# javahedi/SpinDynamics.jl

Hardware: AMD Instinct MI355X
Metric: H|psi> matvecs/s, XXZ L=32 Sz=0 (higher is better)
Workload: dtype c128

## Files before the change

profiles/l2_model.py:

```python
#!/usr/bin/env python3
import os
import sys
from collections import OrderedDict
from math import comb

import numpy as np

L = int(sys.argv[1]) if len(sys.argv) > 1 else 28
orders = sys.argv[2:] or ["lex", "chunk", "orbit"]
LS, nup = int(os.environ.get("LS", "12")), L // 2
p = L - LS
CAP = int(float(os.environ.get("CAP_MIB", "4")) * (1 << 20))
W = int(os.environ.get("W", "160"))
LO, HI = int(os.environ.get("LO", "513")), int(os.environ.get("HI", "1024"))


def tile_len(P):
    return comb(LS, nup - bin(P).count("1")) if 0 <= nup - bin(P).count("1") <= LS else 0


def n_up_first(P):
    t = nup - bin(P).count("1")
    return comb(LS - 1, t - 1) if t >= 1 else 0


all_tiles = [P for P in range(1 << p) if LO <= tile_len(P) <= HI]


def canon(P, FO, greedy):
    C0, member, ng, b = P, 0, 0, 1
    while b + 1 <= p and ng < FO:
        if ((P >> (b - 1)) ^ (P >> b)) & 1:
            if not (P >> (b - 1)) & 1:
                C0 ^= 3 << (b - 1)
                member |= 1 << ng
            ng += 1
            b += 2
        else:
            b += 1 if greedy else 2
    return C0, member


def order_orbit(tiles, FO=6, greedy=False, OC=1, gray=False):
    first, keys = {}, []
    for P in tiles:
        C0, mem = canon(P, FO, greedy)
        if C0 not in first:
            first[C0] = len(first)
        if gray:
            mem = mem ^ (mem >> 1)
        keys.append((first[C0], mem))
    idx = sorted(range(len(tiles)), key=lambda k: keys[k])
    q = [[] for _ in range(8)]
    o, k = 0, 0
    while k < len(idx):
        e = k
        while e < len(idx) and keys[idx[e]][0] == keys[idx[k]][0]:
            e += 1
        q[(o // OC) % 8].extend(tiles[i] for i in idx[k:e])
        o += 1
        k = e
    return q


def order_chunk(tiles, CH=32):
    q = [[] for _ in range(8)]
    for c in range(0, len(tiles), CH):
        q[(c // CH) % 8].extend(tiles[c:c + CH])
    return q


def order_lex(tiles):
    return [tiles[x::8] for x in range(8)]


def events(queue):
    ev = []
    life = 1.0
    for j, P in enumerate(queue):
        t0 = j * life / W
        reads = [((P, 0), n_up_first(P) * 16), ((P, 1), (tile_len(P) - n_up_first(P)) * 16)]
        for b in range(1, p):
            if ((P >> (b - 1)) ^ (P >> b)) & 1:
                Q = P ^ (3 << (b - 1))
                reads.append(((Q, 0), n_up_first(Q) * 16))
                reads.append(((Q, 1), (tile_len(Q) - n_up_first(Q)) * 16))
        Q = P ^ (1 << (p - 1))
        if tile_len(Q) > 0:
            half = 0 if (P >> (p - 1)) & 1 else 1
            sz = n_up_first(Q) * 16 if half == 0 else (tile_len(Q) - n_up_first(Q)) * 16
            if sz > 0:
                reads.append(((Q, half), sz))
        n = len(reads)
        for k, (obj, sz) in enumerate(reads):
            ev.append((t0 + life * (k // 2) / (n // 2 + 1), obj, sz))
    return ev


class LRU:
    def __init__(self, cap):
        self.cap, self.used, self.d = cap, 0, OrderedDict()

    def access(self, obj, sz):
        if obj in self.d:
            self.d.move_to_end(obj)
            return True
        self.d[obj] = sz
        self.used += sz
        while self.used > self.cap:
            _, s2 = self.d.popitem(last=False)
            self.used -= s2
        return False


def simulate(queue):
    ev = events(queue)
    ev.sort(key=lambda e: e[0])
    l2, req, miss = LRU(CAP), 0, 0
    for _, obj, sz in ev:
        req += sz
        if not l2.access(obj, sz):
            miss += sz
    return req, miss


def simulate_all(queues, mall_bytes):
    ev = []
    for x, q in enumerate(queues):
        ev.extend((t, x, obj, sz) for (t, obj, sz) in events(q))
    ev.sort(key=lambda e: e[0])
    l2 = [LRU(CAP) for _ in queues]
    mall = LRU(mall_bytes)
    req = m2 = m3 = 0
    for _, x, obj, sz in ev:
        req += sz
        if l2[x].access(obj, sz):
            continue
        m2 += sz
        if not mall.access(obj, sz):
            m3 += sz
    return req, m2, m3


def parse(name):
    if name == "lex":
        return order_lex(all_tiles)
    if name.startswith("chunk"):
        return order_chunk(all_tiles, int(name[5:] or 32))
    if name.startswith("orbit") or name.startswith("greedy") or name.startswith("gray"):
        kind = "greedy" if name.startswith("greedy") else ("gray" if name.startswith("gray") else "orbit")
        rest = name[len(kind):]
        FO, OC = 6, 1
        if rest:
            parts = rest.split("x")
            FO = int(parts[0])
            if len(parts) > 1:
                OC = int(parts[1])
        return order_orbit(all_tiles, FO, kind == "greedy", OC, kind == "gray")
    raise SystemExit("unknown order " + name)


print(f"L={L} p={p} tiles in class: {len(all_tiles)}  rows: {sum(tile_len(P) for P in all_tiles)}")
MALL = float(os.environ.get("MALL_MIB", "0"))
for name in orders:
    q = parse(name)
    if MALL > 0:
        r, m2, m3 = simulate_all(q, int(MALL * (1 << 20)))
        rows = sum(tile_len(P) for x in q for P in x)
        print(f"{name:12s} read requests {r / rows:6.1f} B/row   L2 misses {m2 / rows:6.1f} B/row   memory-side misses {m3 / rows:6.1f} B/row", flush=True)
        continue
    tot_req = tot_miss = 0
    for x in (0, 3):
        r, m_ = simulate(q[x])
        tot_req += r
        tot_miss += m_
    rows = sum(tile_len(P) for P in q[0]) + sum(tile_len(P) for P in q[3])
    print(f"{name:12s} read requests {tot_req / rows:6.1f} B/row   L2 misses {tot_miss / rows:6.1f} B/row   hit {1 - tot_miss / tot_req:.3f}", flush=True)
```

spindynamics.jl_amd/csrc/basis.cpp:

```cpp
#include <algorithm>
#include <cmath>
#include <cstdlib>
#include <cstring>

#include "sd_internal.hpp"

int64_t sd_binom(int n, int k) {
  if (k < 0 || k > n || n < 0) return 0;
  if (k > n - k) k = n - k;
  __int128 r = 1;
  for (int i = 1; i <= k; ++i) r = r * (n - k + i) / i;
  return (int64_t)r;
}

void sd_fill_binom(std::vector<int64_t> &tab) {
  const int W = SD_MAX_L + 1;
  tab.assign((size_t)W * W, 0);
  for (int n = 0; n < W; ++n)
    for (int k = 0; k <= n; ++k) tab[(size_t)n * W + k] = sd_binom(n, k);
}

static inline int64_t B(const sd_model *m, int n, int k) {
  if (k < 0 || n < 0 || k > n) return 0;
  return m->binom[(size_t)n * (SD_MAX_L + 1) + k];
}

uint64_t sd_unrank_host(const sd_model *m, int64_t idx0) {
  if (m->nup < 0) return (uint64_t)idx0;
  uint64_t s = 0;
  int r = m->nup;
  for (int k = 1; k <= m->L && r > 0; ++k) {
    int64_t c = B(m, m->L - k, r - 1);
    if (idx0 < c) { s |= (uint64_t)1 << (k - 1); --r; }
    else idx0 -= c;
  }
  return s;
}

int64_t sd_rank_host(const sd_model *m, uint64_t s) {
  if (m->L < 64 && (s >> m->L) != 0) return -1;
  if (m->nup < 0) return (int64_t)s;
  if (__builtin_popcountll(s) != m->nup) return -1;
  int64_t idx = 0;
  int r = m->nup;
  for (int k = 1; k <= m->L && r > 0; ++k) {
    if ((s >> (k - 1)) & 1) --r;
    else idx += B(m, m->L - k, r - 1);
  }
  return idx;
}

static void enum_sector(int n, int t, std::vector<uint16_t> &out) {
  if (t < 0 || t > n) return;
  std::vector<int> c(t);
  for (int k = 0; k < t; ++k) c[k] = k + 1;
  for (;;) {
    uint32_t s = 0;
    for (int k = 0; k < t; ++k) s |= 1u << (c[k] - 1);
    out.push_back((uint16_t)s);
    int k = t - 1;
    while (k >= 0 && c[k] == n - t + k + 1) --k;
    if (k < 0) break;
    ++c[k];
    for (int q = k + 1; q < t; ++q) c[q] = c[q - 1] + 1;
  }
}

static int suffix_bits_from_env() {
  int ls = 12;
  if (const char *e = getenv("SD_SUFFIX_BITS")) ls = atoi(e);
  if (ls < 2) ls = 2;
  if (ls > 15) ls = 15;
  return ls;
}

static int64_t tile_base_global(const sd_model *m, uint32_t P) {
  int64_t idx = 0;
  int r = m->nup;
  for (int k = 1; k <= m->p && r > 0; ++k) {
    if ((P >> (k - 1)) & 1) --r;
    else idx += B(m, m->L - k, r - 1);
  }
  return idx;
}

struct TileRef { int64_t base; uint32_t P; };

static void collect_needs(const sd_model *m, const std::vector<TileRef> &tiles, const std::vector<int> &owner, int q,
                          int nn_hops, std::vector<uint8_t> &need) {
  const int p = m->p;
  for (size_t k = 0; k < tiles.size(); ++k) {
    if (owner[k] != q) continue;
    uint32_t P = tiles[k].P;
    if (nn_hops > 0) {
      for (int b = 1; b <= p - 1; ++b)
        if (((P >> (b - 1)) & 1) != ((P >> b) & 1)) need[P ^ (3u << (b - 1))] = 1;
      if (p >= 1) {
        uint32_t Q = P ^ (1u << (p - 1));
        int t2 = m->nup - __builtin_popcount(Q);
        if (t2 >= 0 && t2 <= m->LS) need[Q] = 1;
      }
    }
    for (size_t h = (size_t)nn_hops; h < m->hop_i.size(); ++h) {
      int i = m->hop_i[h], j = m->hop_j[h];
      bool ip = i <= p, jp = j <= p;
      uint32_t Q = P;
      if (ip && jp) {
        if (((P >> (i - 1)) & 1) == ((P >> (j - 1)) & 1)) continue;
        Q = P ^ (1u << (i - 1)) ^ (1u << (j - 1));
      } else if (ip) Q = P ^ (1u << (i - 1));
      else if (jp) Q = P ^ (1u << (j - 1));
      else continue;
      int t2 = m->nup - __builtin_popcount(Q);
      if (t2 >= 0 && t2 <= m->LS) need[Q] = 1;
    }
  }
}

static int count_nn_hops(const sd_model *m) {
  int L = m->L;
  if (L < 2 || (int)m->hop_i.size() < L - 1) return 0;
  for (int k = 0; k < L - 1; ++k)
    if (m->hop_i[k] != k + 1 || m->hop_j[k] != k + 2) return 0;
  return L - 1;
}

static const int XCD_FO_CLASSES = 5, XCD_FO_PACKED = 6;
static std::vector<std::vector<size_t>> xcd_queues(const sd_model *m, int p, const std::vector<uint32_t> &tp_io,
                                                   std::vector<int64_t> &first_seen, const int FO) {
  std::vector<std::vector<size_t>> q(8);
  {
    const int CH = 32;
    const size_t nt = tp_io.size();
    auto canon = [&](uint32_t P, int *member_out) {
      uint32_t C0 = P; int member = 0, ng = 0;
      for (int b = 1; b + 1 <= p && ng < FO; b += 2)
        if (((P >> (b - 1)) ^ (P >> b)) & 1u) {
          if (!((P >> (b - 1)) & 1u)) { C0 ^= 3u << (b - 1); member |= 1 << ng; }
          ++ng;
        }
      if (member_out) *member_out = member;
      return C0;
    };
    auto first_seen_reset = [&](uint32_t P) { first_seen[canon(P, nullptr)] = -1; };
    if (nt >= 64 && p >= 3 && count_nn_hops(m) > 0) {
      std::vector<uint64_t> key(nt);
      int64_t n_orb = 0;
      for (size_t k = 0; k < nt; ++k) {
        int member = 0;
        const uint32_t C0 = canon(tp_io[k], &member);
        if (first_seen[C0] < 0) first_seen[C0] = n_orb++;
        key[k] = ((uint64_t)first_seen[C0] << 8) | (uint64_t)member;
      }
      std::vector<size_t> idx(nt);
      for (size_t k = 0; k < nt; ++k) idx[k] = k;
      std::stable_sort(idx.begin(), idx.end(), [&](size_t a, size_t b) { return key[a] < key[b]; });
      size_t o = 0;
      for (size_t k = 0; k < nt;) {
        size_t e = k;
        while (e < nt && (key[idx[e]] >> 8) == (key[idx[k]] >> 8)) ++e;
        for (size_t t = k; t < e; ++t) q[o % 8].push_back(idx[t]);
        ++o; k = e;
      }
      for (size_t k = 0; k < nt; ++k) first_seen_reset(tp_io[k]);
    } else {
      const size_t group = (size_t)8 * CH, full = nt >= (size_t)16 * CH ? nt / group * group : 0;
      for (size_t b = 0; b < nt; ++b) {
        size_t t = b;
        if (b < full) {
          const size_t x = b % 8, sl = b / 8, g = sl / CH, i = sl % CH;
          t = g * group + x * CH + i;
        }
        q[b % 8].push_back(t);
      }
    }
  }
  return q;
}

static void xcd_order(const sd_model *m, int p, std::vector<uint32_t> &tp_io, std::vector<int64_t> &tb_io,
                      std::vector<int64_t> &first_seen) {
  const std::vector<std::vector<size_t>> q = xcd_queues(m, p, tp_io, first_seen, XCD_FO_CLASSES);
  const size_t nt = tp_io.size();
  std::vector<uint32_t> tp; std::vector<int64_t> tb;
  tp.reserve(nt); tb.reserve(nt);
  size_t longest = 0;
  for (auto &v : q) longest = std::max(longest, v.size());
  for (size_t j = 0; j < longest; ++j)
    for (int x = 0; x < 8; ++x)
      if (j < q[x].size()) { tp.push_back(tp_io[q[x][j]]); tb.push_back(tb_io[q[x][j]]); }
  tp_io.swap(tp); tb_io.swap(tb);
}

struct BisectPlan {
  int d = 0;
  int s[4] = {0, 0, 0, 0};
  int thr[3][4] = {{0}};
  double score = 1e300;
  double busiest = 0;
};

static int bisect_owner(const BisectPlan &bp, const int *k) {
  int cum[4] = {0, 0, 0, 0};
  for (int i = 0; i < bp.d; ++i) cum[i + 1] = cum[i] + k[i];
  int r = 0;
  for (int lev = 0; lev < bp.d; ++lev) r = 2 * r + (cum[bp.d - lev] > bp.thr[lev][r] ? 1 : 0);
  return r;
}

static bool eval_bisect(const sd_model *m, BisectPlan &bp) {
  const int d = bp.d, L = m->L, nup = m->nup, P = 1 << d;
  int len[3] = {0, 0, 0};
  for (int i = 0; i < d; ++i) len[i] = bp.s[i + 1] - bp.s[i];
  const int rest = L - bp.s[d];
  auto weight = [&](const int *k) {
    int sum = 0; double w = 1;
    for (int i = 0; i < d; ++i) { w *= (double)B(m, len[i], k[i]); sum += k[i]; }
    return w * (double)B(m, rest, nup - sum);
  };
  auto for_cells = [&](auto &&fn) {
    int k[3] = {0, 0, 0};
    for (k[0] = 0; k[0] <= len[0]; ++k[0])
      for (k[1] = 0; k[1] <= (d > 1 ? len[1] : 0); ++k[1])
        for (k[2] = 0; k[2] <= (d > 2 ? len[2] : 0); ++k[2]) fn(k);
  };
  for (int lev = 0; lev < d; ++lev)
    for (int pre = 0; pre < (1 << lev); ++pre) {
      const int blk = d - lev;
      std::vector<double> hist(bp.s[blk] + 1, 0.0);
      double tot = 0;
      for_cells([&](const int *k) {
        int cum[4] = {0, 0, 0, 0};
        for (int i = 0; i < d; ++i) cum[i + 1] = cum[i] + k[i];
        int r = 0;
        for (int q = 0; q < lev; ++q) r = 2 * r + (cum[d - q] > bp.thr[q][r] ? 1 : 0);
        if (r != pre) return;
        const double w = weight(k);
        hist[cum[blk]] += w; tot += w;
      });
      if (tot <= 0) return false;
      double acc = 0, bestd = 1e300; int t = 0;
      for (int v = 0; v < bp.s[blk]; ++v) {
        acc += hist[v];
        const double dd = std::fabs(acc - tot / 2);
        if (dd < bestd) { bestd = dd; t = v; }
      }
      bp.thr[lev][pre] = t;
    }
  std::vector<double> size(P, 0.0), vol(P, 0.0), pair((size_t)P * P, 0.0);
  for_cells([&](const int *k) {
    int sum = 0;
    for (int i = 0; i < d; ++i) sum += k[i];
    const int kr = nup - sum;
    if (kr < 0 || kr > rest) return;
    const int me = bisect_owner(bp, k);
    size[me] += weight(k);
    for (int i = 0; i < d; ++i) {
      const bool last = i == d - 1;
      const int lr = last ? rest : len[i + 1], kright = last ? kr : k[i + 1];
      double others = 1;
      for (int q = 0; q < d; ++q) if (q != i && (last || q != i + 1)) others *= (double)B(m, len[q], k[q]);
      if (!last) others *= (double)B(m, rest, kr);
      for (int dir = 0; dir < 2; ++dir) {
        const double n = dir == 0 ? (double)B(m, len[i] - 1, k[i] - 1) * (double)B(m, lr - 1, kright) * others
                                  : (double)B(m, len[i] - 1, k[i]) * (double)B(m, lr - 1, kright - 1) * others;
        if (n <= 0) continue;
        int k2[3] = {k[0], k[1], k[2]};
        k2[i] += dir == 0 ? -1 : 1;
        if (!last) k2[i + 1] += dir == 0 ? 1 : -1;
        const int o = bisect_owner(bp, k2);
        if (o != me) { vol[me] += n; pair[(size_t)me * P + o] += n; }
      }
    }
  });
  double tot = 0;
  for (int r = 0; r < P; ++r) tot += size[r];
  bp.score = 0; bp.busiest = 0;
  for (int r = 0; r < P; ++r) {
    if (size[r] <= 0 || size[r] > 1.15 * tot / P) return false;
    bp.score = std::max(bp.score, vol[r] / size[r]);
  }
  for (double v : pair) bp.busiest = std::max(bp.busiest, v);
  return true;
}

static bool best_bisect_plan(const sd_model *m, int p, int nranks, BisectPlan &best) {
  int d = 0;
  while ((1 << d) < nranks) ++d;
  if ((1 << d) != nranks || d < 1 || d > 3 || m->nup < 0) return false;
  bool found = false;
  BisectPlan bp; bp.d = d;
  for (int s1 = 2; s1 <= p - 1; ++s1)
    for (int s2 = (d > 1 ? s1 + 2 : s1); s2 <= (d > 1 ? p - 1 : s1); ++s2)
      for (int s3 = (d > 2 ? s2 + 2 : s2); s3 <= (d > 2 ? p - 1 : s2); ++s3) {
        bp.s[0] = 0; bp.s[1] = s1; bp.s[2] = s2; bp.s[3] = s3;
        if (!eval_bisect(m, bp)) continue;
        if (!found || bp.score < best.score * (1 - 1e-12) ||
            (bp.score <= best.score * (1 + 1e-12) && bp.busiest < best.busiest)) { best = bp; found = true; }
      }
  return found;
}

int sd_build_plan(sd_model *m, int rank, int nranks, std::string &err) {
  if (nranks < 1 || rank < 0 || rank >= nranks) { err = "bad shard rank/nranks"; return SD_EARG; }
  m->rank = rank; m->nranks = nranks;
  m->tile_prefix.clear(); m->tile_base.clear(); m->addr.clear();
  m->suf_states.clear(); m->suf_rank.clear(); m->suf_off.clear(); m->suf_part.clear();
  m->recv_slabs.clear(); m->send_slabs.clear();
  m->n_halo = 0; m->max_tile_len = 0;
  m->n_short = 0; m->short_off = 0; m->n_short_multi = 0;

  const int L = m->L;
  int LS = std::min(L, suffix_bits_from_env());
  if (m->nup >= 0) {
    auto longest = [&](int ls) {
      int64_t mx = 0;
      for (int t = std::max(0, m->nup - (L - ls)); t <= std::min(ls, m->nup); ++t) mx = std::max(mx, B(m, ls, t));
      return mx;
    };
    while (LS > 2 && longest(LS) > 4096) --LS;
  }
  int p = L - LS;
  m->max_tile_len_all = 0;
  if (m->nup >= 0)
    for (int t = std::max(0, m->nup - (L - LS)); t <= std::min(LS, m->nup); ++t)
      m->max_tile_len_all = std::max<int>(m->max_tile_len_all, (int)std::min<int64_t>(B(m, LS, t), 1 << 30));
  bool short_tiles = false;
  if (m->nup >= 0 && p >= 0 && p <= SD_MAX_PREFIX_BITS && nranks == 1) {
    double nt = 0;
    for (int k = std::max(0, m->nup - LS); k <= std::min(p, m->nup); ++k) nt += (double)B(m, p, k);
    short_tiles = nt > 0 && (double)m->N / nt < 32.0 && p >= 1 && m->N < 1500000;
  }
  if (m->nup < 0 || p > SD_MAX_PREFIX_BITS || short_tiles) {
    m->p = -1; m->LS = 0;
    m->row_lo = 0; m->row_hi = m->N; m->n_local = m->N;
    m->shard_mode = 0; m->n_interior = 0; m->fs_dbits = 0;
    m->pack_src.clear(); m->pack_dst.clear(); m->pack_len.clear(); m->n_send = 0;
    m->full_ls = (m->nup < 0 && L >= 12 && L <= 40) ? 10 : 0;
    if (nranks == 1) return SD_OK;
    int d = 0;
    while ((1 << d) < nranks) ++d;
    const int nnh = count_nn_hops(m);
    if (m->nup >= 0) { err = "sharding needs a fixed-nup sector with at most 2^26 prefix tiles, or the full basis"; return SD_EARG; }
    if ((1 << d) != nranks || nranks > SD_FS_MAX_RANKS) { err = "the full 2^L basis shards over 2, 4 or 8 ranks (top index bits)"; return SD_EARG; }
    if (m->full_ls == 0 || L - d < m->full_ls + 1) { err = "full-basis sharding needs L >= 12 and at least two tiles per rank"; return SD_EARG; }
    if (nnh == 0 || (int)m->hop_i.size() != nnh) { err = "full-basis sharding needs the open chain's hop list (bonds (i, i+1) in order)"; return SD_EARG; }
    m->fs_dbits = d;
    m->n_local = m->N / nranks;
    m->row_lo = (int64_t)rank * m->n_local; m->row_hi = m->row_lo + m->n_local;
    for (int q = 0; q < SD_FS_MAX_RANKS; ++q) { m->fs_halo_off[q] = -1; m->fs_peer_lo[q] = 0; }
    int64_t hoff = 0;
    auto add_pair = [&](int me, int peer, int64_t peer_lo, int64_t count, bool recv) {
      if (recv) {
        m->fs_halo_off[peer] = hoff; m->fs_peer_lo[peer] = peer_lo;
        m->recv_slabs.push_back({peer, m->n_local + hoff, count, (int64_t)peer * m->n_local + peer_lo});
        hoff += count;
      } else {
        m->send_slabs.push_back({peer, peer_lo, count, (int64_t)me * m->n_local + peer_lo});
      }
    };
    add_pair(rank, rank ^ 1, (int64_t)(rank & 1) * (m->n_local / 2), m->n_local / 2, true);
    for (int k = 0; k + 1 < d; ++k)
      if (((rank >> k) ^ (rank >> (k + 1))) & 1) add_pair(rank, rank ^ (3 << k), 0, m->n_local, true);
    add_pair(rank, rank ^ 1, (int64_t)((rank ^ 1) & 1) * (m->n_local / 2), m->n_local / 2, false);
    for (int k = 0; k + 1 < d; ++k)
      if (((rank >> k) ^ (rank >> (k + 1))) & 1) add_pair(rank, rank ^ (3 << k), 0, m->n_local, false);
    m->n_halo = hoff;
    return SD_OK;
  }
  m->p = p; m->LS = LS; m->full_ls = 0;

  m->suf_off.assign(LS + 2, 0);
  m->suf_rank.assign((size_t)1 << LS, 0);
  for (int t = 0; t <= LS; ++t) {
    m->suf_off[t] = (int32_t)m->suf_states.size();
    enum_sector(LS, t, m->suf_states);
    int32_t n = (int32_t)m->suf_states.size() - m->suf_off[t];
    for (int32_t i = 0; i < n; ++i) m->suf_rank[m->suf_states[m->suf_off[t] + i]] = (uint16_t)i;
  }
  m->suf_off[LS + 1] = (int32_t)m->suf_states.size();
  m->suf_part.clear(); m->suf_dg.clear();
  m->wrap_hop = -1;
  if (LS <= 12) {
    m->suf_part.assign(4 * m->suf_states.size(), 0u);
    m->suf_dg.assign(m->suf_states.size(), 0);
    const uint32_t inner = LS >= 2 ? ((1u << (LS - 1)) - 1u) : 0u;
    for (size_t k = 0; k < m->suf_states.size(); ++k) {
      const uint32_t sg = m->suf_states[k];
      uint32_t *w = m->suf_part.data() + 4 * k;
      for (int a = 1; a <= LS - 1; ++a)
        if (((sg >> (a - 1)) ^ (sg >> a)) & 1u) {
          const uint32_t partner = (uint32_t)m->suf_rank[sg ^ (3u << (a - 1))] + 1u;
          w[(a - 1) / 3] |= partner << (10 * ((a - 1) % 3));
        }
      m->suf_dg[k] = (uint8_t)(__builtin_popcount((sg ^ (sg >> 1)) & inner) | ((sg & 1u) << 4));
    }
    m->wrap_hop = -1;
    const int nnh = count_nn_hops(m);
    if (nnh > 0 && nnh < (int)m->hop_i.size() && p >= 1) {
      const int bi = m->hop_i[nnh] - 1, bj = m->hop_j[nnh] - 1;
      if ((bi < p) != (bj < p)) {
        const int sb = (bi < p ? bj : bi) - p;
        m->wrap_hop = nnh; m->wrap_pb = bi < p ? bi : bj;
        for (int t = 0; t <= LS; ++t)
          for (int32_t i = m->suf_off[t]; i < m->suf_off[t + 1]; ++i) {
            const uint32_t sg = m->suf_states[i];
            const bool up = (sg >> sb) & 1u;
            const int tq = up ? t - 1 : t + 1;
            uint32_t field = 0;
            if (tq >= 0 && tq <= LS) field = (uint32_t)m->suf_rank[sg ^ (1u << sb)] + 1u;
            m->suf_part[4 * (size_t)i + 3] |= (field << 20) | ((up ? 1u : 0u) << 30);
          }
      }
    }
  }

  std::vector<TileRef> tiles;
  const uint32_t nP = 1u << p;
  for (uint32_t P = 0; P < nP; ++P) {
    int t2 = m->nup - __builtin_popcount(P);
    if (t2 < 0 || t2 > LS) continue;
    tiles.push_back({tile_base_global(m, P), P});
  }
  std::sort(tiles.begin(), tiles.end(), [](const TileRef &a, const TileRef &b) { return a.base < b.base; });
  const size_t T = tiles.size();
  if (T == 0) { err = "empty basis"; return SD_EINTERNAL; }

  std::vector<int> owner(T, 0);
  std::vector<int64_t> tlen(T);
  for (size_t k = 0; k < T; ++k) tlen[k] = B(m, LS, m->nup - __builtin_popcount(tiles[k].P));
  int mode = m->shard_mode_req;
  if (mode < 0) {
    mode = 1;
    if (const char *e = getenv("SD_SHARD_MODE")) mode = (e[0] == 'r') ? 0 : 1;
  }
  if (nranks == 1 || count_nn_hops(m) == 0 || p < 6) mode = 0;
  if (mode == 1) {
    double best = 1e300; int bm1 = -1, bm2 = -1; std::vector<int> bassign;
    for (int m1 = 4; m1 <= p - 1; ++m1)
      for (int m2 = 2; m2 <= m1 - 2; ++m2) {
        const int W2 = m2 + 1;
        std::vector<double> w((size_t)(m1 + 1) * W2, 0.0);
        double tot = 0;
        for (int k1 = 0; k1 <= m1; ++k1)
          for (int k2 = 0; k2 <= std::min(k1, m2); ++k2) {
            const double x = (double)B(m, m2, k2) * (double)B(m, m1 - m2, k1 - k2) * (double)B(m, L - m1, m->nup - k1);
            w[(size_t)k1 * W2 + k2] = x; tot += x;
          }
        std::vector<int> assign((size_t)(m1 + 1) * W2, -1);
        std::vector<double> size(nranks, 0.0), vol(nranks, 0.0);
        double acc = 0; int r = 0;
        for (size_t c = 0; c < w.size(); ++c) {
          if (w[c] == 0) continue;
          if (acc + w[c] / 2 > (r + 1) * tot / nranks && r < nranks - 1) ++r;
          assign[c] = r; acc += w[c]; size[r] += w[c];
        }
        bool ok = true;
        for (int q = 0; q < nranks; ++q) if (size[q] == 0 || size[q] > 1.15 * tot / nranks) ok = false;
        if (!ok) continue;
        auto A = [&](int k1, int k2) { return (k1 < 0 || k1 > m1 || k2 < 0 || k2 > m2 || k2 > k1) ? -1 : assign[(size_t)k1 * W2 + k2]; };
        for (int k1 = 0; k1 <= m1; ++k1)
          for (int k2 = 0; k2 <= std::min(k1, m2); ++k2) {
            const int rr = A(k1, k2);
            if (rr < 0) continue;
            const double rest = (double)B(m, L - m1, m->nup - k1);
            auto add = [&](double n, int other) { if (n > 0 && other >= 0 && other != rr) vol[rr] += n; };
            add((double)B(m, m2 - 1, k2 - 1) * (double)B(m, m1 - m2 - 1, k1 - k2) * rest, A(k1, k2 - 1));
            add((double)B(m, m2 - 1, k2) * (double)B(m, m1 - m2 - 1, k1 - k2 - 1) * rest, A(k1, k2 + 1));
            add((double)B(m, m2, k2) * (double)B(m, m1 - m2 - 1, k1 - k2 - 1) * (double)B(m, L - m1 - 1, m->nup - k1), A(k1 - 1, k2));
            add((double)B(m, m2, k2) * (double)B(m, m1 - m2 - 1, k1 - k2) * (double)B(m, L - m1 - 1, m->nup - k1 - 1), A(k1 + 1, k2));
          }
        double score = 0;
        for (int q = 0; q < nranks; ++q) score = std::max(score, vol[q] / size[q]);
        if (score < best) { best = score; bm1 = m1; bm2 = m2; bassign = assign; }
      }
    BisectPlan bis;
    const bool have_bis = best_bisect_plan(m, p, nranks, bis);
    if (have_bis && (bm1 < 0 || bis.score < best)) {
      for (size_t k = 0; k < T; ++k) {
        int cnt[3] = {0, 0, 0};
        for (int i = 0; i < bis.d; ++i) {
          const uint32_t lo = bis.s[i] == 0 ? 0u : ((1u << bis.s[i]) - 1u), hi = (1u << bis.s[i + 1]) - 1u;
          cnt[i] = __builtin_popcount(tiles[k].P & (hi & ~lo));
        }
        owner[k] = bisect_owner(bis, cnt);
      }
      const int K = 3;
      std::vector<int> fine(T, 0);
      std::vector<int32_t> idx_of((size_t)nP, -1);
      for (size_t k = 0; k < T; ++k) idx_of[tiles[k].P] = (int32_t)k;
      for (int lev = 0; lev < bis.d; ++lev) {
        const int sb = bis.s[bis.d - lev], kk = std::min(K, p - sb);
        const uint32_t bmask = (1u << sb) - 1u;
        auto zof = [&](uint32_t P) {
          uint32_t z = (uint32_t)__builtin_popcount(P & bmask);
          for (int j = 0; j < kk; ++j) z = 2 * z + ((P >> (sb + j)) & 1u);
          return z;
        };
        const size_t nz = ((size_t)sb + 1) << kk;
        std::vector<double> hist((size_t)(1 << lev) * nz, 0.0);
        for (size_t k = 0; k < T; ++k) hist[(size_t)fine[k] * nz + zof(tiles[k].P)] += (double)tlen[k];
        std::vector<uint32_t> thr((size_t)1 << lev, 0);
        for (int pre = 0; pre < (1 << lev); ++pre) {
          const double *h = hist.data() + (size_t)pre * nz;
          double tot = 0; for (size_t z = 0; z < nz; ++z) tot += h[z];
          double acc = 0, bestd = 1e300;
          for (size_t z = 0; z + 1 < nz; ++z) {
            acc += h[z];
            const double dd = std::fabs(acc - tot / 2);
            if (dd < bestd) { bestd = dd; thr[pre] = (uint32_t)z; }
          }
        }
        for (size_t k = 0; k < T; ++k) fine[k] = 2 * fine[k] + (zof(tiles[k].P) > thr[fine[k]] ? 1 : 0);
      }
      auto judge = [&](const std::vector<int> &own, double &crossing, double &largest) {
        crossing = 0;
        std::vector<double> size(nranks, 0.0);
        for (size_t k = 0; k < T; ++k) {
          const uint32_t P = tiles[k].P;
          size[own[k]] += (double)tlen[k];
          for (int b = 1; b <= p - 1; ++b)
            if (((P >> (b - 1)) ^ (P >> b)) & 1u) {
              const int32_t j = idx_of[P ^ (3u << (b - 1))];
              if (j >= 0 && own[j] != own[k]) crossing += (double)tlen[j];
            }
        }
        largest = 0;
        bool empty = false;
        for (double v : size) { largest = std::max(largest, v); if (v <= 0) empty = true; }
        return !empty;
      };
      double c0 = 0, l0 = 0, c1 = 0, l1 = 0;
      judge(owner, c0, l0);
      const bool ok1 = judge(fine, c1, l1);
      if (ok1 && l1 < l0 && c1 <= 1.05 * c0) owner.swap(fine);
    } else if (bm1 < 0) mode = 0;
    else {
      const uint32_t mA = (1u << bm1) - 1, mB = (1u << bm2) - 1;
      for (size_t k = 0; k < T; ++k)
        owner[k] = bassign[(size_t)__builtin_popcount(tiles[k].P & mA) * (bm2 + 1) + __builtin_popcount(tiles[k].P & mB)];
    }
  }
  if (mode == 0) {
    for (int r = 1; r < nranks; ++r) {
      const int64_t target = (int64_t)((__int128)m->N * r / nranks);
      for (size_t k = 0; k < T; ++k) if (tiles[k].base >= target) owner[k] = std::max(owner[k], r);
    }
  }
  m->shard_mode = mode;

  std::vector<int64_t> local_of(T, -1);
  m->addr.assign(nP, -1);
  m->row_lo = -1; m->row_hi = 0; m->n_local = 0;
  for (size_t k = 0; k < T; ++k) {
    if (owner[k] != rank) continue;
    if (m->row_lo < 0) m->row_lo = tiles[k].base;
    m->row_hi = tiles[k].base + tlen[k];
    local_of[k] = m->n_local;
    m->tile_prefix.push_back(tiles[k].P);
    m->tile_base.push_back(m->n_local);
    m->addr[tiles[k].P] = m->n_local;
    m->n_local += tlen[k];
    m->max_tile_len = std::max<int>(m->max_tile_len, (int)tlen[k]);
  }
  if (m->row_lo < 0) {
    m->row_lo = m->row_hi = m->N;
    for (size_t k = 0; k < T; ++k)
      if (owner[k] > rank) { m->row_lo = m->row_hi = tiles[k].base; break; }
  }

  std::vector<int64_t> xcd_scratch((size_t)1 << p, -1);
  xcd_order(m, p, m->tile_prefix, m->tile_base, xcd_scratch);

  m->single_prefix = m->tile_prefix; m->single_base = m->tile_base;

  m->pack_src.clear(); m->pack_dst.clear(); m->pack_len.clear(); m->n_send = 0;
  m->packed = 0;
  if (nranks > 1) {
    const int nn = count_nn_hops(m);
    std::vector<uint8_t> need(nP);
    std::vector<int64_t> nloc(nranks, 0);
    std::vector<int64_t> loc_all(T, 0);
    for (size_t k = 0; k < T; ++k) { loc_all[k] = nloc[owner[k]]; nloc[owner[k]] += tlen[k]; }
    std::vector<sd_slab> d_recv, d_send;
    int64_t n_runs_all = 0, n_rows_all = 0;
    for (int q = 0; q < nranks; ++q) {
      std::fill(need.begin(), need.end(), 0);
      collect_needs(m, tiles, owner, q, nn, need);
      int64_t halo_off = nloc[q];
      if (mode == 0) {
        sd_slab cur{-1, 0, 0, 0};
        int64_t cur_end_global = -1;
        auto flush = [&]() { if (cur.count && q == rank) m->recv_slabs.push_back(cur); cur.count = 0; };
        for (size_t k = 0; k < T; ++k) {
          if (!need[tiles[k].P] || owner[k] == q) continue;
          const int own = owner[k];
          const int64_t len = tlen[k];
          if (q == rank) {
            m->addr[tiles[k].P] = halo_off;
            if (cur.count > 0 && cur.peer == own && cur_end_global == tiles[k].base) cur.count += len;
            else { flush(); cur = {own, halo_off, len, tiles[k].base}; }
            cur_end_global = tiles[k].base + len;
          } else if (own == rank) {
            const int64_t loc = local_of[k];
            if (!m->send_slabs.empty() && m->send_slabs.back().peer == q &&
                m->send_slabs.back().local_offset + m->send_slabs.back().count == loc)
              m->send_slabs.back().count += len;
            else m->send_slabs.push_back({q, loc, len, tiles[k].base});
          }
          halo_off += len;
        }
        flush();
      } else {
        for (int o = 0; o < nranks; ++o) {
          if (o == q) continue;
          const int64_t start = halo_off, sstart = m->n_send;
          int64_t count = 0;
          int64_t run_loc = -1, run_halo = 0, run_cnt = 0;
          auto flush_run = [&]() {
            if (run_cnt <= 0) return;
            ++n_runs_all; n_rows_all += run_cnt;
            if (q == rank) d_recv.push_back({o, run_halo, run_cnt, -1});
            if (o == rank) d_send.push_back({q, run_loc, run_cnt, -1});
            run_cnt = 0;
          };
          for (size_t k = 0; k < T; ++k) {
            if (owner[k] != o || !need[tiles[k].P]) continue;
            if (q == rank) m->addr[tiles[k].P] = halo_off;
            if (o == rank) { m->pack_src.push_back(local_of[k]); m->pack_dst.push_back(m->n_send); m->pack_len.push_back((int32_t)tlen[k]); m->n_send += tlen[k]; }
            if (run_cnt > 0 && loc_all[k] == run_loc + run_cnt) run_cnt += tlen[k];
            else { flush_run(); run_loc = loc_all[k]; run_halo = halo_off; run_cnt = tlen[k]; }
            halo_off += tlen[k]; count += tlen[k];
          }
          flush_run();
          if (count > 0) {
            if (q == rank) m->recv_slabs.push_back({o, start, count, -1});
            if (o == rank) m->send_slabs.push_back({q, sstart, count, -1});
          }
        }
      }
      if (q == rank) m->n_halo = halo_off - m->n_local;
    }
    if (mode == 1) {
      const char *fp = getenv("SD_SHARD_PACK");
      const bool direct = fp ? atoi(fp) == 0 : (n_runs_all > 0 && n_rows_all / n_runs_all >= 2048);
      if (direct) {
        m->recv_slabs.swap(d_recv); m->send_slabs.swap(d_send);
        m->pack_src.clear(); m->pack_dst.clear(); m->pack_len.clear(); m->n_send = 0;
      } else m->packed = 1;
    }
  }
  {
    const size_t ns = m->single_prefix.size();
    std::vector<uint8_t> boundary(ns, 0);
    if (nranks > 1 && m->n_halo > 0) {
      const int nn = count_nn_hops(m);
      auto remote = [&](uint32_t Q) { return Q < nP && m->addr[Q] >= m->n_local; };
      for (size_t k = 0; k < ns; ++k) {
        const uint32_t P = m->single_prefix[k];
        bool bd = false;
        if (nn > 0) {
          for (int b = 1; b <= p - 1 && !bd; ++b)
            if ((((P >> (b - 1)) ^ (P >> b)) & 1u) && remote(P ^ (3u << (b - 1)))) bd = true;
          if (!bd && p >= 1 && remote(P ^ (1u << (p - 1)))) bd = true;
        }
        for (size_t h = (size_t)nn; h < m->hop_i.size() && !bd; ++h) {
          const int i = m->hop_i[h], j = m->hop_j[h];
          uint32_t Q = P;
          if (i <= p) Q ^= 1u << (i - 1);
          if (j <= p) Q ^= 1u << (j - 1);
          if (Q != P && remote(Q)) bd = true;
        }
        boundary[k] = bd;
      }
    }
    bool split = ns >= 32768;
    if (const char *e = getenv("SD_LEN_CLASSES")) split = atoi(e) >= 2 || (split && atoi(e) != 0);
    int top = 0;
    while (top < SD_N_LEN_CLASS - 1 && (64 << top) * 4 < m->max_tile_len) ++top;
    if (m->LS > 12) { split = false; top = std::max(top, 3); }
    auto cls_of = [&](uint32_t P) {
      if (!split) return top;
      const int64_t len = B(m, m->LS, m->nup - __builtin_popcount(P));
      int c = 0;
      while (c < top && (64 << c) * 4 < len) ++c;
      return c;
    };
    std::vector<std::vector<uint32_t>> sp(2 * SD_N_LEN_CLASS);
    std::vector<std::vector<int64_t>> sb(2 * SD_N_LEN_CLASS);
    std::vector<uint32_t> short_p; std::vector<int64_t> short_b;
    bool use_short = false;
    if (nranks == 1 && m->LS <= 12 && p >= 1) {
      size_t n_sh = 0;
      for (size_t k = 0; k < ns; ++k) if (B(m, m->LS, m->nup - __builtin_popcount(m->single_prefix[k])) <= 16) ++n_sh;
      use_short = n_sh >= 8192 && 5 * n_sh >= ns;
      if (const char *e = getenv("SD_SHORT_TILES")) use_short = atoi(e) != 0 && n_sh > 0;
    }
    for (size_t k = 0; k < ns; ++k) {
      if (use_short && B(m, m->LS, m->nup - __builtin_popcount(m->single_prefix[k])) <= 16) {
        short_p.push_back(m->single_prefix[k]); short_b.push_back(m->single_base[k]);
        continue;
      }
      const int sgi = boundary[k] * SD_N_LEN_CLASS + (SD_N_LEN_CLASS - 1 - cls_of(m->single_prefix[k]));
      sp[sgi].push_back(m->single_prefix[k]); sb[sgi].push_back(m->single_base[k]);
    }
    m->single_prefix.clear(); m->single_base.clear();
    for (int sgi = 0; sgi < 2 * SD_N_LEN_CLASS; ++sgi) {
      m->seg_off[sgi] = (int)m->single_prefix.size();
      m->seg_cls[sgi] = SD_N_LEN_CLASS - 1 - sgi % SD_N_LEN_CLASS;
      if (split || (nranks > 1 && m->n_halo > 0)) xcd_order(m, p, sp[sgi], sb[sgi], xcd_scratch);
      m->single_prefix.insert(m->single_prefix.end(), sp[sgi].begin(), sp[sgi].end());
      m->single_base.insert(m->single_base.end(), sb[sgi].begin(), sb[sgi].end());
    }
    m->seg_off[2 * SD_N_LEN_CLASS] = (int)m->single_prefix.size();
    m->n_interior = m->seg_off[SD_N_LEN_CLASS];
    m->short_off = (int)m->single_prefix.size(); m->n_short = (int)short_p.size(); m->n_short_multi = 0;
    for (int pass = 0; pass < 2; ++pass)
      for (size_t k = 0; k < short_p.size(); ++k) {
        const bool one = B(m, m->LS, m->nup - __builtin_popcount(short_p[k])) == 1;
        if (one != (pass == 1)) continue;
        m->single_prefix.push_back(short_p[k]); m->single_base.push_back(short_b[k]);
        if (pass == 0) ++m->n_short_multi;
      }
    m->blk_tiles.clear();
    bool pack = nranks == 1 && split && m->LS <= 12 && p >= 1 && m->short_off > 0;
    if (pack) {
      const char *e = getenv("SD_LEN_CLASSES");
      if (!(e && atoi(e) >= 2)) {
        int64_t rows_one = 0, rows_all = 0;
        for (int k = 0; k < m->short_off; ++k) {
          const int64_t len = B(m, m->LS, m->nup - __builtin_popcount(m->single_prefix[k]));
          rows_all += len;
          if (len <= 256) rows_one += len;
        }
        pack = 8 * rows_one <= rows_all;
      }
    }
    if (pack) {
      std::vector<int32_t> index_of((size_t)1 << p, -1);
      for (int k = 0; k < m->short_off; ++k) index_of[m->single_prefix[k]] = k;
      std::vector<std::pair<int64_t, uint32_t>> by_base((size_t)m->short_off);
      for (int k = 0; k < m->short_off; ++k) by_base[k] = {m->single_base[k], m->single_prefix[k]};
      std::sort(by_base.begin(), by_base.end());
      std::vector<uint32_t> all((size_t)m->short_off);
      for (int k = 0; k < m->short_off; ++k) all[k] = by_base[k].second;
      const std::vector<std::vector<size_t>> q = xcd_queues(m, p, all, xcd_scratch, XCD_FO_PACKED);
      auto slots_of = [&](uint32_t P) { return (int)((B(m, m->LS, m->nup - __builtin_popcount(P)) + 255) / 256); };
      std::vector<std::vector<int32_t>> qb(8);
      for (int x = 0; x < 8; ++x) {
        int used = 4;
        for (size_t t : q[x]) {
          const int ns_t = slots_of(all[t]);
          if (ns_t < 1 || ns_t > 4) { err = "block table: tile longer than a workgroup"; return SD_EINTERNAL; }
          if (used + ns_t > 4) { qb[x].insert(qb[x].end(), 4, -1); used = 0; }
          for (int s = 0; s < ns_t; ++s) qb[x][qb[x].size() - 4 + (size_t)(used + s)] = index_of[all[t]];
          used += ns_t;
        }
      }
      size_t longest = 0;
      for (auto &v : qb) longest = std::max(longest, v.size() / 4);
      for (size_t j = 0; j < longest; ++j)
        for (int x = 0; x < 8; ++x)
          if (j < qb[x].size() / 4) m->blk_tiles.insert(m->blk_tiles.end(), qb[x].begin() + 4 * j, qb[x].begin() + 4 * j + 4);
      std::vector<int32_t> seen((size_t)m->short_off, 0);
      bool ok = true;
      for (size_t b = 0; b < m->blk_tiles.size() / 4 && ok; ++b) {
        const int32_t *bt = m->blk_tiles.data() + 4 * b;
        for (int s = 0; s < 4 && ok; ++s) {
          const int32_t t = bt[s];
          if (t == -1) continue;
          if (t < 0 || t >= m->short_off) { ok = false; break; }
          if (s > 0 && bt[s - 1] == t) continue;
          int run = 1;
          while (s + run < 4 && bt[s + run] == t) ++run;
          for (int s2 = s + run; s2 < 4; ++s2) if (bt[s2] == t) ok = false;
          if (seen[t] != 0 || run != slots_of(m->single_prefix[t])) ok = false;
          seen[t] = 1;
        }
      }
      for (int k = 0; k < m->short_off && ok; ++k) if (!seen[k]) ok = false;
      if (!ok) { m->blk_tiles.clear(); err = "block table of the packed launch failed its self-check"; return SD_EINTERNAL; }
    }
  }
  m->tile_gbase.resize(m->tile_prefix.size());
  for (size_t k = 0; k < m->tile_prefix.size(); ++k) m->tile_gbase[k] = tile_base_global(m, m->tile_prefix[k]);
  return SD_OK;
}

static bool exact_multiples(double q, int n) {
  for (int k = 1; k <= n; ++k)
    if (std::fma((double)k, q, -((double)k * q)) != 0.0) return false;
  return true;
}

template <class T>
static int up(sd_model *m, const std::vector<T> &v, const T **dst, std::string &err) {
  *dst = nullptr;
  size_t bytes = sizeof(T) * std::max<size_t>(v.size(), 1);
  void *d = nullptr;
  hipError_t e = hipMalloc(&d, bytes);
  if (e != hipSuccess) { err = std::string("hipMalloc: ") + hipGetErrorString(e); return SD_ENOMEM; }
  m->dev_allocs.push_back(d);
  if (!v.empty()) {
    e = hipMemcpy(d, v.data(), sizeof(T) * v.size(), hipMemcpyHostToDevice);
    if (e != hipSuccess) { err = std::string("hipMemcpy: ") + hipGetErrorString(e); return SD_EHIP; }
  }
  *dst = (const T *)d;
  return SD_OK;
}

void sd_free_device_tables(sd_model *m) {
  for (void *d : m->dev_allocs) (void)hipFree(d);
  m->dev_allocs.clear();
  m->dev_ready = false;
}

int sd_upload_model(sd_model *m, std::string &err) {
  sd_free_device_tables(m);
  sd_dev_model &d = m->dm;
  memset(&d, 0, sizeof(d));
  d.L = m->L; d.nup = m->nup; d.p = m->p; d.LS = m->LS;
  d.n_hop = (int)m->hop_i.size(); d.n_zz = (int)m->zz_i.size();
  d.N = m->N; d.n_local = m->n_local; d.row_lo = m->row_lo;
  d.full_ls = m->full_ls;
  d.fs_dbits = m->fs_dbits;
  for (int q = 0; q < SD_FS_MAX_RANKS; ++q) { d.fs_halo_off[q] = m->fs_halo_off[q]; d.fs_peer_lo[q] = m->fs_peer_lo[q]; }
  d.nn_hops = (m->p >= 0 || m->full_ls > 0 || m->nup >= 0) ? count_nn_hops(m) : 0;
  d.field_zero = 1;
  for (double h : m->field) if (h != 0.0) d.field_zero = 0;
  d.diag_mode = 0; d.diag_q = 0.0; d.n_zz_nn = 0;
  if (d.field_zero) {
    bool uniform = true;
    for (double J : m->zz_J) if (J != m->zz_J[0]) uniform = false;
    if (m->zz_J.empty()) { d.diag_mode = 1; d.diag_q = 0.0; }
    else if (uniform) {
      double q = (m->zz_J[0] * 0.5) * 0.5;
      if (exact_multiples(q, (int)m->zz_J.size())) { d.diag_mode = 1; d.diag_q = q; }
    }
  }
  if (m->L >= 2 && (int)m->zz_i.size() >= m->L - 1) {
    bool nn = true;
    for (int k = 0; k < m->L - 1; ++k)
      if (m->zz_i[k] != k + 1 || m->zz_j[k] != k + 2) nn = false;
    if (nn) d.n_zz_nn = m->L - 1;
  }
  m->zz_q.resize(m->zz_J.size());
  for (size_t k = 0; k < m->zz_J.size(); ++k) m->zz_q[k] = (m->zz_J[k] * 0.5) * 0.5;
  m->field_h.resize(m->field.size());
  for (size_t k = 0; k < m->field.size(); ++k) m->field_h[k] = m->field[k] * 0.5;
  m->hop_pow2 = true;
  for (int k = 0; k < d.nn_hops; ++k) {
    int ex; const double mant = std::frexp(m->hop_J[k], &ex);
    if (!(m->hop_J[k] == 0.0 || std::fabs(mant) == 0.5) || !std::isfinite(m->hop_J[k])) m->hop_pow2 = false;
  }
  int rc;
  if ((rc = up(m, m->hop_i, &d.hop_i, err))) return rc;
  if ((rc = up(m, m->hop_j, &d.hop_j, err))) return rc;
  if ((rc = up(m, m->hop_J, &d.hop_J, err))) return rc;
  if ((rc = up(m, m->zz_i, &d.zz_i, err))) return rc;
  if ((rc = up(m, m->zz_j, &d.zz_j, err))) return rc;
  if ((rc = up(m, m->zz_q, &d.zz_q, err))) return rc;
  if ((rc = up(m, m->field_h, &d.field_h, err))) return rc;
  if ((rc = up(m, m->binom, &d.binom, err))) return rc;
  d.n_tiles = (int)m->tile_prefix.size();
  if (m->p >= 0) {
    if ((rc = up(m, m->tile_prefix, &d.tile_prefix, err))) return rc;
    if ((rc = up(m, m->tile_base, &d.tile_base, err))) return rc;
    if ((rc = up(m, m->addr, &d.addr, err))) return rc;
    if ((rc = up(m, m->suf_states, &d.suf_states, err))) return rc;
    if ((rc = up(m, m->suf_off, &d.suf_off, err))) return rc;
    if ((rc = up(m, m->suf_rank, &d.suf_rank, err))) return rc;
    if (!m->suf_part.empty()) {
      if ((rc = up(m, m->suf_part, &d.suf_part, err))) return rc;
      if ((rc = up(m, m->suf_dg, &d.suf_dg, err))) return rc;
    } else { d.suf_part = nullptr; d.suf_dg = nullptr; }
    d.wrap_hop = m->suf_part.empty() ? -1 : m->wrap_hop; d.wrap_pb = m->wrap_pb;
    if ((rc = up(m, m->tile_gbase, &d.tile_gbase, err))) return rc;
    d.n_pack = (int)m->pack_len.size();
    if ((rc = up(m, m->pack_src, &d.pack_src, err))) return rc;
    if ((rc = up(m, m->pack_dst, &d.pack_dst, err))) return rc;
    if ((rc = up(m, m->pack_len, &d.pack_len, err))) return rc;
    d.n_singles = (int)m->single_prefix.size();
    d.n_interior = m->n_interior; d.tile_off = 0;
    d.n_short = m->n_short; d.short_off = m->short_off; d.n_short_multi = m->n_short_multi;
    d.n_blk = 0; d.blk_tiles = nullptr;
    m->single_rec.resize(m->single_prefix.size());
    for (size_t k = 0; k < m->single_prefix.size(); ++k) {
      const uint32_t P = m->single_prefix[k];
      const int t2 = m->nup - __builtin_popcount(P);
      sd_tile_rec &r = m->single_rec[k];
      r.base = m->single_base[k]; r.prefix = P;
      r.len = (int32_t)B(m, m->LS, t2); r.nU = (int32_t)B(m, m->LS - 1, t2 - 1); r.suf_off = m->suf_off[t2];
      r.pad0 = r.pad1 = 0;
    }
    if ((rc = up(m, m->single_rec, &d.single_rec, err))) return rc;
    {
      const int p = m->p, LS = m->LS;
      m->far_base.clear();
      m->far_base.shrink_to_fit();
      if (p >= 1 && d.nn_hops > 0) m->far_base.assign(m->single_prefix.size() * (size_t)p, -1);
      if (p >= 1 && d.nn_hops > 0)
        for (size_t k = 0; k < m->single_prefix.size(); ++k) {
          const uint32_t P = m->single_prefix[k];
          int64_t *fb = m->far_base.data() + k * (size_t)p;
          for (int b = 1; b <= p - 1; ++b)
            if (((P >> (b - 1)) ^ (P >> b)) & 1u) fb[b - 1] = m->addr[P ^ (3u << (b - 1))];
          const uint32_t bitp = (P >> (p - 1)) & 1u, Q = P ^ (1u << (p - 1));
          const int t2 = m->nup - __builtin_popcount(P), t2q = m->nup - __builtin_popcount(Q);
          if (t2q >= 0 && t2q <= LS) {
            const int64_t len = B(m, LS, t2), nU = B(m, LS - 1, t2 - 1), nUq = B(m, LS - 1, t2q - 1);
            const int64_t my_n = bitp ? len - nU : nU;
            if (my_n > 0) fb[p - 1] = m->addr[Q] + (bitp ? 0 : nUq);
          }
        }
      if ((rc = up(m, m->far_base, &d.far_base, err))) return rc;
    }
    if ((rc = up(m, m->single_prefix, &d.single_prefix, err))) return rc;
    if ((rc = up(m, m->single_base, &d.single_base, err))) return rc;
    m->gen.clear(); m->gen_ss_part.clear(); m->mix_part.clear();
    d.n_gen = 0; d.n_gen_mixed = 0; d.n_suf_rows = (int)m->suf_states.size();
    d.gen = nullptr; d.gen_ss_part = nullptr; d.mix_part = nullptr;
    {
      const int p = m->p, LS = m->LS, nn = d.nn_hops;
      const char *ge = getenv("SD_GEN_PLAN");
      const bool wrap_only = d.n_hop == nn + 1 && d.wrap_hop == nn && !(ge && atoi(ge) == 2);
      if (!m->suf_part.empty() && d.n_hop > nn && !wrap_only && !(ge && atoi(ge) == 0)) {
        const size_t nsr = m->suf_states.size();
        int n_ss = 0;
        std::vector<int> mix_site(LS, 0);
        for (int h = nn; h < d.n_hop; ++h) {
          const int bi = m->hop_i[h] - 1, bj = m->hop_j[h] - 1;
          sd_gbond g{-1, 0u, 0, 0, m->hop_J[h]};
          if (bi != bj) {
            const bool ip = bi < p, jp = bj < p;
            if (ip && jp) { g.kind = 0; g.pmask = (1u << bi) | (1u << bj); }
            else if (!ip && !jp) { g.kind = 1; g.pmask = (1u << (bi - p)) | (1u << (bj - p)); g.slot = n_ss++; }
            else { g.kind = 2; g.pb = ip ? bi : bj; g.pmask = 1u << g.pb; g.slot = (ip ? bj : bi) - p; mix_site[g.slot] = 1; ++d.n_gen_mixed; }
          }
          m->gen.push_back(g);
        }
        const int n_chunks = (n_ss + 11) / 12;
        m->gen_ss_part.assign((size_t)std::max(n_chunks, 1) * nsr * 4, 0u);
        for (const sd_gbond &g : m->gen)
          if (g.kind == 1) {
            const int chunk = g.slot / 12, f = g.slot % 12;
            for (size_t k = 0; k < nsr; ++k) {
              const uint32_t sg = m->suf_states[k];
              if (__builtin_popcount(sg & g.pmask) != 1) continue;
              const uint32_t partner = (uint32_t)m->suf_rank[sg ^ g.pmask] + 1u;
              m->gen_ss_part[((size_t)chunk * nsr + k) * 4 + (size_t)(f / 3)] |= partner << (10 * (f % 3));
            }
          }
        m->mix_part.assign((size_t)LS * nsr, 0);
        for (int sb = 0; sb < LS; ++sb)
          if (mix_site[sb])
            for (size_t k = 0; k < nsr; ++k) {
              const uint32_t sg = m->suf_states[k];
              m->mix_part[(size_t)sb * nsr + k] = (uint16_t)(((uint32_t)m->suf_rank[sg ^ (1u << sb)] + 1u) | (((sg >> sb) & 1u) << 15));
            }
        for (sd_gbond &g : m->gen) if (g.kind == 1) g.pmask = 0u;
        if ((rc = up(m, m->gen, &d.gen, err))) return rc;
        if ((rc = up(m, m->gen_ss_part, &d.gen_ss_part, err))) return rc;
        if ((rc = up(m, m->mix_part, &d.mix_part, err))) return rc;
        d.n_gen = (int)m->gen.size();
        d.wrap_hop = -1;
      }
    }
    if (!m->blk_tiles.empty() && d.suf_part && d.wrap_hop < 0 && d.n_gen == 0) {
      if ((rc = up(m, m->blk_tiles, &d.blk_tiles, err))) return rc;
      d.n_blk = (int)(m->blk_tiles.size() / 4);
    }
  }
  const char *dc_env = getenv("SD_DIAG_CACHE");
  if (m->p >= 0 && d.diag_mode == 0 && d.n_local > 0 && d.n_tiles > 0 && !(dc_env && atoi(dc_env) == 0)) {
    void *dc = nullptr;
    if (hipMalloc(&dc, sizeof(double) * (size_t)d.n_local) == hipSuccess) {
      m->dev_allocs.push_back(dc);
      if (sd_k_build_diag(d, (double *)dc) == SD_OK) d.diag_cache = (const double *)dc;
    } else {
      (void)hipGetLastError();
    }
  }
  {
    const bool chain_diag = d.diag_mode == 1 && (d.n_zz == 0 || (d.n_zz_nn == m->L - 1 && d.n_zz == d.n_zz_nn));
    d.need_sig = (d.n_hop > d.nn_hops) || !(d.diag_cache || chain_diag) || !d.suf_part;
    d.need_sig_gen = !(d.diag_cache || chain_diag);
  }
  m->dev_ready = true;
  return SD_OK;
}
```

Before: 96.69.

## Group packed tiles into larger quad/pair orbits and deal orbits by row count

Generalizes the tile orbit key used to order work across the eight XCD queues. Four-bit quad blocks are canonicalized in addition to adjacent-pair flips, under a member-bit budget. Packed tiles whose neighbouring prefixes share vector data are grouped on the same XCD so their reads hit that XCD's L2. Orbits are now dealt to whichever queue has the fewest rows rather than round-robin, to balance load. The risk is larger orbits that reduce balance or exceed L2 capacity, and the key width changes to 16 bits.

```diff
diff --git a/profiles/l2_model.py b/profiles/l2_model.py
--- a/profiles/l2_model.py
+++ b/profiles/l2_model.py
@@ -4,7 +4,8 @@
 from collections import OrderedDict
 from math import comb
 
-import numpy as np
+sys.path.insert(0, os.path.dirname(os.path.abspath(__file__)))
+from orbit_key import orbit_key
 
 L = int(sys.argv[1]) if len(sys.argv) > 1 else 28
 orders = sys.argv[2:] or ["lex", "chunk", "orbit"]
@@ -24,7 +25,21 @@
     return comb(LS - 1, t - 1) if t >= 1 else 0
 
 
+def tile_base(P):
+    idx, r = 0, nup
+    for k in range(1, p + 1):
+        if r <= 0:
+            break
+        if (P >> (k - 1)) & 1:
+            r -= 1
+        else:
+            idx += comb(L - k, r - 1)
+    return idx
+
+
 all_tiles = [P for P in range(1 << p) if LO <= tile_len(P) <= HI]
+if os.environ.get("ASC", "0") == "1":
+    all_tiles.sort(key=tile_base)
 
 
 def canon(P, FO, greedy):
@@ -41,10 +56,13 @@
     return C0, member
 
 
-def order_orbit(tiles, FO=6, greedy=False, OC=1, gray=False):
+def order_orbit(tiles, FO=6, greedy=False, OC=1, gray=False, block=None, deal_rows=False):
     first, keys = {}, []
     for P in tiles:
-        C0, mem = canon(P, FO, greedy)
+        if block:
+            C0, mem, _ = orbit_key(P, p, block[0], block[1])
+        else:
+            C0, mem = canon(P, FO, greedy)
         if C0 not in first:
             first[C0] = len(first)
         if gray:
@@ -52,14 +70,20 @@
         keys.append((first[C0], mem))
     idx = sorted(range(len(tiles)), key=lambda k: keys[k])
     q = [[] for _ in range(8)]
-    o, k = 0, 0
+    rows = [0] * 8
+    o, k, largest = 0, 0, 0
     while k < len(idx):
         e = k
         while e < len(idx) and keys[idx[e]][0] == keys[idx[k]][0]:
             e += 1
-        q[(o // OC) % 8].extend(tiles[i] for i in idx[k:e])
+        x = rows.index(min(rows)) if deal_rows else (o // OC) % 8
+        q[x].extend(tiles[i] for i in idx[k:e])
+        rows[x] += sum(tile_len(tiles[i]) for i in idx[k:e])
+        largest = max(largest, e - k)
         o += 1
         k = e
+    print(f"  orbits {o}  largest {largest} tiles  rows per queue {rows}"
+          f"  max - min {(max(rows) - min(rows)) / (sum(rows) / 8) * 100:.3f} % of the mean")
     return q
 
 
@@ -147,6 +171,10 @@
         return order_lex(all_tiles)
     if name.startswith("chunk"):
         return order_chunk(all_tiles, int(name[5:] or 32))
+    if name.startswith("block"):
+        deal = name.endswith("d")
+        B_, C_ = name[5:].rstrip("d").split("c")
+        return order_orbit(all_tiles, block=(int(B_), int(C_)), deal_rows=deal)
     if name.startswith("orbit") or name.startswith("greedy") or name.startswith("gray"):
         kind = "greedy" if name.startswith("greedy") else ("gray" if name.startswith("gray") else "orbit")
         rest = name[len(kind):]
diff --git a/profiles/orbit_key.py b/profiles/orbit_key.py
--- /dev/null
+++ b/profiles/orbit_key.py
@@ -0,0 +1,43 @@
+
+QUAD_COUNT = (1, 4, 6, 4, 1)
+QUAD_MBITS = (0, 2000, 2585, 2000, 0)
+
+
+def orbit_key(P, p, quad_blocks, cap_tenths):
+    cap = 100 * cap_tenths
+    rep, member, mult, used, moves = P, 0, 1, 0, []
+    b = 1
+    while b + 1 <= p:
+        if b % 4 == 1 and (b - 1) // 4 < quad_blocks and b + 3 <= p:
+            cfg = (P >> (b - 1)) & 15
+            k = bin(cfg).count("1")
+            if QUAD_COUNT[k] > 1 and used + QUAD_MBITS[k] <= cap:
+                digit = sum(1 for c in range(cfg) if bin(c).count("1") == k)
+                rep = (rep & ~(15 << (b - 1))) | (((1 << k) - 1) << (b - 1))
+                member += digit * mult
+                mult *= QUAD_COUNT[k]
+                used += QUAD_MBITS[k]
+                moves.append(("quad", b, k))
+                b += 4
+                continue
+        if ((P >> (b - 1)) ^ (P >> b)) & 1 and used + 1000 <= cap:
+            if not (P >> (b - 1)) & 1:
+                rep ^= 3 << (b - 1)
+                member += mult
+            mult *= 2
+            used += 1000
+            moves.append(("pair", b))
+        b += 2
+    return rep, member, moves
+
+
+def neighbours(P, moves):
+    out = []
+    for mv in moves:
+        if mv[0] == "pair":
+            out.append(P ^ (3 << (mv[1] - 1)))
+        else:
+            _, b, k = mv
+            cur = (P >> (b - 1)) & 15
+            out.extend((P & ~(15 << (b - 1))) | (c << (b - 1)) for c in range(16) if bin(c).count("1") == k and c != cur)
+    return out
diff --git a/spindynamics.jl_amd/csrc/basis.cpp b/spindynamics.jl_amd/csrc/basis.cpp
--- a/spindynamics.jl_amd/csrc/basis.cpp
+++ b/spindynamics.jl_amd/csrc/basis.cpp
@@ -3,6 +3,7 @@
 #include <cstdlib>
 #include <cstring>
 
+#include "orbit_key.hpp"
 #include "sd_internal.hpp"
 
 int64_t sd_binom(int n, int k) {
@@ -125,22 +126,28 @@
   return L - 1;
 }
 
-static const int XCD_FO_CLASSES = 5, XCD_FO_PACKED = 6;
+#ifndef SD_ORBIT_QUAD_BLOCKS
+#define SD_ORBIT_QUAD_BLOCKS 2
+#endif
+#ifndef SD_ORBIT_CAP_TENTHS
+#define SD_ORBIT_CAP_TENTHS 78
+#endif
+#ifndef SD_ORBIT_DEAL_ROWS
+#define SD_ORBIT_DEAL_ROWS 1
+#endif
+static_assert(SD_ORBIT_QUAD_BLOCKS >= 0 && SD_ORBIT_CAP_TENTHS >= 0 && SD_ORBIT_CAP_TENTHS <= 150, "orbit member ids take 16 key bits");
+struct OrbitRule { int quad_blocks, cap_tenths; bool deal_rows; };
+static const OrbitRule XCD_RULE_CLASSES = {0, 50, false}, XCD_RULE_PACKED = {SD_ORBIT_QUAD_BLOCKS, SD_ORBIT_CAP_TENTHS, SD_ORBIT_DEAL_ROWS != 0};
 static std::vector<std::vector<size_t>> xcd_queues(const sd_model *m, int p, const std::vector<uint32_t> &tp_io,
-                                                   std::vector<int64_t> &first_seen, const int FO) {
+                                                   std::vector<int64_t> &first_seen, const OrbitRule rule) {
   std::vector<std::vector<size_t>> q(8);
   {
     const int CH = 32;
     const size_t nt = tp_io.size();
     auto canon = [&](uint32_t P, int *member_out) {
-      uint32_t C0 = P; int member = 0, ng = 0;
-      for (int b = 1; b + 1 <= p && ng < FO; b += 2)
-        if (((P >> (b - 1)) ^ (P >> b)) & 1u) {
-          if (!((P >> (b - 1)) & 1u)) { C0 ^= 3u << (b - 1); member |= 1 << ng; }
-          ++ng;
-        }
-      if (member_out) *member_out = member;
-      return C0;
+      const sd_orbit_key o = sd_orbit_key_of(P, p, rule.quad_blocks, rule.cap_tenths);
+      if (member_out) *member_out = (int)o.member;
+      return o.rep;
     };
     auto first_seen_reset = [&](uint32_t P) { first_seen[canon(P, nullptr)] = -1; };
     if (nt >= 64 && p >= 3 && count_nn_hops(m) > 0) {
@@ -150,16 +157,23 @@
         int member = 0;
         const uint32_t C0 = canon(tp_io[k], &member);
         if (first_seen[C0] < 0) first_seen[C0] = n_orb++;
-        key[k] = ((uint64_t)first_seen[C0] << 8) | (uint64_t)member;
+        key[k] = ((uint64_t)first_seen[C0] << 16) | (uint64_t)member;
       }
       std::vector<size_t> idx(nt);
       for (size_t k = 0; k < nt; ++k) idx[k] = k;
       std::stable_sort(idx.begin(), idx.end(), [&](size_t a, size_t b) { return key[a] < key[b]; });
       size_t o = 0;
+      int64_t q_rows[8] = {0, 0, 0, 0, 0, 0, 0, 0};
       for (size_t k = 0; k < nt;) {
         size_t e = k;
-        while (e < nt && (key[idx[e]] >> 8) == (key[idx[k]] >> 8)) ++e;
-        for (size_t t = k; t < e; ++t) q[o % 8].push_back(idx[t]);
+        while (e < nt && (key[idx[e]] >> 16) == (key[idx[k]] >> 16)) ++e;
+        size_t x = o % 8;
+        if (rule.deal_rows) {
+          x = 0;
+          for (size_t y = 1; y < 8; ++y) if (q_rows[y] < q_rows[x]) x = y;
+        }
+        for (size_t t = k; t < e; ++t) q[x].push_back(idx[t]);
+        q_rows[x] += (int64_t)(e - k) * B(m, m->LS, m->nup - __builtin_popcount(tp_io[idx[k]]));
         ++o; k = e;
       }
       for (size_t k = 0; k < nt; ++k) first_seen_reset(tp_io[k]);
@@ -180,7 +194,7 @@
 
 static void xcd_order(const sd_model *m, int p, std::vector<uint32_t> &tp_io, std::vector<int64_t> &tb_io,
                       std::vector<int64_t> &first_seen) {
-  const std::vector<std::vector<size_t>> q = xcd_queues(m, p, tp_io, first_seen, XCD_FO_CLASSES);
+  const std::vector<std::vector<size_t>> q = xcd_queues(m, p, tp_io, first_seen, XCD_RULE_CLASSES);
   const size_t nt = tp_io.size();
   std::vector<uint32_t> tp; std::vector<int64_t> tb;
   tp.reserve(nt); tb.reserve(nt);
@@ -744,7 +758,7 @@
       std::sort(by_base.begin(), by_base.end());
       std::vector<uint32_t> all((size_t)m->short_off);
       for (int k = 0; k < m->short_off; ++k) all[k] = by_base[k].second;
-      const std::vector<std::vector<size_t>> q = xcd_queues(m, p, all, xcd_scratch, XCD_FO_PACKED);
+      const std::vector<std::vector<size_t>> q = xcd_queues(m, p, all, xcd_scratch, XCD_RULE_PACKED);
       auto slots_of = [&](uint32_t P) { return (int)((B(m, m->LS, m->nup - __builtin_popcount(P)) + 255) / 256); };
       std::vector<std::vector<int32_t>> qb(8);
       for (int x = 0; x < 8; ++x) {
diff --git a/spindynamics.jl_amd/csrc/orbit_key.hpp b/spindynamics.jl_amd/csrc/orbit_key.hpp
--- /dev/null
+++ b/spindynamics.jl_amd/csrc/orbit_key.hpp
@@ -0,0 +1,33 @@
+#pragma once
+#include <cstdint>
+
+struct sd_orbit_key { uint32_t rep, member; };
+
+static inline sd_orbit_key sd_orbit_key_of(uint32_t P, int p, int quad_blocks, int cap_tenths) {
+  static const int quad_count[5] = {1, 4, 6, 4, 1}, quad_mbits[5] = {0, 2000, 2585, 2000, 0};
+  const int cap = 100 * cap_tenths;
+  sd_orbit_key o = {P, 0};
+  uint32_t mult = 1;
+  int used = 0;
+  for (int b = 1; b + 1 <= p;) {
+    if (b % 4 == 1 && (b - 1) / 4 < quad_blocks && b + 3 <= p) {
+      const uint32_t cfg = (P >> (b - 1)) & 15u;
+      const int k = __builtin_popcount(cfg);
+      if (quad_count[k] > 1 && used + quad_mbits[k] <= cap) {
+        uint32_t digit = 0;
+        for (uint32_t c = 0; c < cfg; ++c) digit += __builtin_popcount(c) == k;
+        o.rep = (o.rep & ~(15u << (b - 1))) | (((1u << k) - 1u) << (b - 1));
+        o.member += digit * mult; mult *= (uint32_t)quad_count[k];
+        used += quad_mbits[k];
+        b += 4;
+        continue;
+      }
+    }
+    if ((((P >> (b - 1)) ^ (P >> b)) & 1u) && used + 1000 <= cap) {
+      if (!((P >> (b - 1)) & 1u)) { o.rep ^= 3u << (b - 1); o.member += mult; }
+      mult *= 2; used += 1000;
+    }
+    b += 2;
+  }
+  return o;
+}
```

New measurement: 101.2, median of 6. +4.7%, better.
